# I2S9/dexterous-rl-manipulation

Hardware: NVIDIA B200
Metric: env_steps_per_sec (higher is better)
Workload: dtype f32+f64

## Files before the change

dexterous_rl_manipulation_b200/csrc/dexsim_kernels.cu:

```cuda
#include <cstdio>
#include <cstdlib>
#include <cstring>
#include <atomic>
#include <mutex>
#include <type_traits>

#include "dexsim_core.cuh"

namespace dexsim {

constexpr int STEP_MIN_BLOCKS = 2;
constexpr int STEP_THREADS = 256;

constexpr int SMEM_GROUPS_MAX = 64;

struct Hot {
    double op_old[3];
    float  ov_old[3];
    unsigned cmask_old;
};

__device__ __forceinline__ void load_env(const DexsimState& st, int64_t i, EnvRegs& e) {
    const int64_t ld = st.ld;
    const float* __restrict__ obs = st.obs;
// ... 80 lines not shown

__device__ __forceinline__ void record_episode(unsigned long long* cnt, double* rs, int success, int steps,
                                               int final_c, int la, int lb, int tie, double ret) {
    atomicAdd(&cnt[DEXSIM_CNT_EPISODES], 1ull);
    if (success) atomicAdd(&cnt[DEXSIM_CNT_SUCCESSES], 1ull);
    atomicAdd(&cnt[DEXSIM_CNT_SUM_STEPS], (unsigned long long)steps);
    atomicAdd(&cnt[DEXSIM_CNT_SUM_STEPS_SQ], (unsigned long long)steps * (unsigned long long)steps);
    if (final_c) atomicAdd(&cnt[DEXSIM_CNT_SUM_FINAL_CONTACTS], (unsigned long long)final_c);
    if (la != DEXSIM_LABEL_NONE) atomicAdd(&cnt[DEXSIM_CNT_LABEL_METRICS + la], 1ull);
    if (lb != DEXSIM_LABEL_NONE) atomicAdd(&cnt[DEXSIM_CNT_LABEL_TAXONOMY + lb], 1ull);
    if (tie == 1) atomicAdd(&cnt[DEXSIM_CNT_VAR_TIES], 1ull);
    if (rs) { atomicAdd(&rs[0], ret); atomicAdd(&rs[1], __dmul_rn(ret, ret)); }
}

struct EpisodeLog {
    DexsimEpisodeRecord* rec = nullptr;
    unsigned long long* count = nullptr;
    long long capacity = 0;
    uint32_t t_end = 0;
};

__device__ __forceinline__ void finish_episode(const EnvRegs& e, const DexsimParams& p, uint32_t gid, uint32_t episode,
                                               double ep_return, const EpStats& es, bool terminated, int n_c,
                                               unsigned long long* cnt, double* rs, const EpisodeLog* log,
                                               const bool classify = true) {
    if (!(cnt || (log && log->rec))) return;
    if (!classify) {
        if (cnt) record_episode(cnt, nullptr, p.success_is_terminated ? (terminated ? 1 : 0) : 0, e.sc, n_c,
                                DEXSIM_LABEL_NONE, DEXSIM_LABEL_NONE, 0, 0.0);
        return;
    }
    DexsimEpisodeSummary s;
    s.success = p.success_is_terminated ? (terminated ? 1 : 0) : 0;
    s.episode_steps = e.sc; s.num_contacts = n_c; s.final_contacts = n_c; s.hist_len = e.sc;
    int sum, sq, f5, l5, mx;
    epstats_unpack(es, sum, sq, f5, l5, mx);
    s.max_count = mx; s.sum_counts = sum; s.sum_sq_counts = sq; s.first5_sum = f5; s.last5_sum = l5;
    int la, lb, tie;
    classify_summary(s, p.loop_max_steps > 0 ? p.loop_max_steps : p.max_episode_steps, p.success_threshold, la, lb, tie);
    if (cnt) record_episode(cnt, rs, s.success, e.sc, n_c, la, lb, tie, ep_return);
    if (log && log->rec) {
        const unsigned long long slot = atomicAdd(log->count, 1ull);
        if ((long long)slot < log->capacity) {
            DexsimEpisodeRecord r;
            r.env_gid = gid; r.episode = episode; r.steps = e.sc;
            r.success = (uint8_t)s.success; r.final_contacts = (uint8_t)n_c;
            r.label_metrics = (uint8_t)la; r.label_taxonomy = (uint8_t)lb;
            r.episode_reward = ep_return; r.t_end = log->t_end; r.var_tie = (uint32_t)tie;
            log->rec[slot] = r;
        }
    }
}

__device__ __forceinline__ void finish_and_reset(EnvRegs& e, const DexsimParams& p, const DexsimGroup& grp,
                                                 uint32_t gid, uint32_t& episode, double& ep_return, EpStats& es,
                                                 bool terminated, int n_c, unsigned long long* cnt, double* rs,
                                                 double& size, double& mass, double& friction,
                                                 const EpisodeLog* log = nullptr, const bool classify = true) {
    finish_episode(e, p, gid, episode, ep_return, es, terminated, n_c, cnt, rs, log, classify);
    episode += 1u;
    float jp0[NJ], pos[3];
    reset_draws(p.seed, gid, episode, grp, jp0, size, mass, friction, pos);
    env_reset(e, jp0, size, friction, pos, !p.respawn);
    ep_return = 0.0;
    es.w0 = 0u; es.w1 = 0u;
}

__device__ __forceinline__ bool pending_reset(const EnvRegs& e, const DexsimParams& p) {
    return e.sc > 0 && (__popc(e.cmask) >= p.success_threshold || e.sc > p.max_episode_steps ||
                        (p.loop_max_steps > 0 && e.sc >= p.loop_max_steps));
}

__device__ __forceinline__ void next_step_reset(EnvRegs& e, const DexsimParams& p, const DexsimGroup& grp, uint32_t gid,
                                                uint32_t& episode, const DexsimState& st, int64_t i, StepResult& r) {
    double ep_return = 0.0, size, mass, friction;
    EpStats es{0u, 0u};
    finish_and_reset(e, p, grp, gid, episode, ep_return, es, false, 0, nullptr, nullptr, size, mass, friction);
    st.episode[i] = episode;
    st.size[i] = size; st.mass[i] = mass; st.friction[i] = friction;
    r.total = r.distance = r.contact = r.closure = r.stability = 0.0;
    r.n_c = __popc(e.cmask);
    r.terminated = r.truncated = false;
}

__device__ __forceinline__ float obs_entry(const EnvRegs& e, const int row) {
    if (row < DEXSIM_ROW_JV) return e.jp[row - DEXSIM_ROW_JP];
    if (row < DEXSIM_ROW_OP) return e.jv[row - DEXSIM_ROW_JV];
    if (row < DEXSIM_ROW_QUAT) return (float)e.op[row - DEXSIM_ROW_OP];
    if (row < DEXSIM_ROW_OV) return row == DEXSIM_ROW_QUAT ? 1.0f : 0.0f;
    if (row < DEXSIM_ROW_CONTACT) return e.ov[row - DEXSIM_ROW_OV];
    return ((e.cmask >> (row - DEXSIM_ROW_CONTACT)) & 1u) ? 1.0f : 0.0f;
}

}

#include "dexsim_step_tma.cuh"
#include "dexsim_rollout_split.cuh"

namespace dexsim {

template <bool TAGGED>
__device__ __forceinline__ void pack_env_body(const DexsimState& st, const DexsimStepIO& io, const int64_t i, const int after_reset,
                                              double* __restrict__ out) {
    const int t = threadIdx.x;
    const int64_t ld = st.ld;
    const bool noisy = io.noisy_obs && (io.obs_noise || io.sigma_obs != 0.0f);
    const float* obs = noisy ? io.noisy_obs : st.obs;
    if (t < NOBS) out[t] = (double)obs[t * ld + i];
    if (t == 45) out[45] = after_reset ? 0.0 : (io.reward64 ? io.reward64[i] : (double)io.reward[i]);
    if (t == 46) out[46] = after_reset ? 0.0 : (double)io.terminated[i];
    if (t == 47) out[47] = after_reset ? 0.0 : (double)io.truncated[i];
    if (t == 48) out[48] = (double)__popc((unsigned)st.cmask[i]);
    if (t == 49) out[49] = (double)st.step_count[i];
    if (t >= 50 && t < 53) out[t] = st.op64[(t - 50) * ld + i];
    if (t == 53) out[53] = st.size[i];
    if (t == 54) out[54] = st.mass[i];
    if (t == 55) out[55] = st.friction[i];
    if (t >= 56 && t < 60) out[t] = (io.reward_comps && !after_reset) ? (double)io.reward_comps[(t - 56) * ld + i] : 0.0;
// ... 700 lines not shown
    }
    if (need_groups) {
        if (p->num_groups < 1 || p->num_groups > DEXSIM_MAX_GROUPS) return DEXSIM_E_GROUPS;
        if (!groups) return DEXSIM_E_NULL;
    }
    return 0;
}

static int grid_for(int64_t n, int threads, int ctas_per_sm, int sm_count) {
    int64_t blocks = (n + threads - 1) / threads;
    const int64_t cap = (int64_t)sm_count * (ctas_per_sm > 0 ? ctas_per_sm : 1);
    if (blocks > cap) blocks = cap;
    if (blocks < 1) blocks = 1;
    return (int)blocks;
}

static inline int cuda_rc(cudaError_t e) { return e == cudaSuccess ? 0 : -(int)e; }

template <bool DENSE, bool AOS>
static void launch_step_variant(bool extras, bool next, int grid, cudaStream_t s, const DexsimState& st, const DexsimParams& p,
                                const DexsimGroup* groups, const uint16_t* goe, const DexsimStepIO& io,
                                double* pack_out, double pack_tag) {
    if (next)        step_kernel<DENSE, AOS, true, true><<<grid, STEP_THREADS, 0, s>>>(st, p, groups, goe, io, pack_out, pack_tag);
    else if (extras) step_kernel<DENSE, AOS, true, false><<<grid, STEP_THREADS, 0, s>>>(st, p, groups, goe, io, pack_out, pack_tag);
    else             step_kernel<DENSE, AOS, false, false><<<grid, STEP_THREADS, 0, s>>>(st, p, groups, goe, io);
}

template <auto KERNEL, typename GridOf, typename... Args>
static int launch_pdl(int threads, size_t smem, GridOf grid_of, cudaStream_t s, const Args&... args) {
    static thread_local int occupancy[64] = {0};
    int dev = 0;
    cudaError_t err = cudaGetDevice(&dev);
    if (err != cudaSuccess) return -(int)err;
    int uncached = 0;
    int& ctas_per_sm = (dev >= 0 && dev < 64) ? occupancy[dev] : uncached;
    if (ctas_per_sm == 0) {
        if (smem) {
            err = cudaFuncSetAttribute(KERNEL, cudaFuncAttributeMaxDynamicSharedMemorySize, (int)smem);
            if (err != cudaSuccess) return -(int)err;
        }
        err = cudaOccupancyMaxActiveBlocksPerMultiprocessor(&ctas_per_sm, KERNEL, threads, smem);
        if (err != cudaSuccess) return -(int)err;
        if (ctas_per_sm < 1) ctas_per_sm = 1;
    }
    cudaLaunchConfig_t cfg = {};
    cfg.gridDim = dim3((unsigned)grid_of(ctas_per_sm)); cfg.blockDim = dim3(threads); cfg.dynamicSmemBytes = smem; cfg.stream = s;
    cudaLaunchAttribute attr[1];
    attr[0].id = cudaLaunchAttributeProgrammaticStreamSerialization;
    attr[0].val.programmaticStreamSerializationAllowed = 1;
    cfg.attrs = attr; cfg.numAttrs = 1;
    return cuda_rc(cudaLaunchKernelEx(&cfg, KERNEL, args...));
}

template <bool DENSE, bool AOS, int TRACK, bool EXTRA, int STAGES, int TILE_, bool NEXT>
static int launch_tma_variant(int sm_count, cudaStream_t s, const DexsimState& st, const DexsimParams& p,
                              const DexsimGroup* groups, const uint16_t* goe, const DexsimStepIO& io,
                              const StepMaps& maps, int num_tiles) {
    constexpr int TMA_THREADS = TILE_ + 32;
    const size_t smem = (size_t)STAGES * StageLayout<TILE_>::stage_bytes(TRACK) + 2 * STAGES * (sizeof(uint64_t) + sizeof(int)) +
                        (TRACK ? TMA_GROUPS_MAX * (DEXSIM_NCOUNTERS * sizeof(unsigned long long) + 2 * sizeof(double)) : 0);
    return launch_pdl<step_tma_kernel<DENSE, AOS, TRACK, EXTRA, STAGES, TILE_, NEXT>>(
        TMA_THREADS, smem, [&](int ctas_per_sm) { return sm_count * ctas_per_sm < num_tiles ? sm_count * ctas_per_sm : num_tiles; }, s,
        st, p, groups, goe, io, maps, num_tiles, 1);
}

static int g_rollout_impl = 0;
static int g_step_impl = 0;

static int g_step_tile = 0;

static bool aligned16(const void* ptr) { return !(reinterpret_cast<uintptr_t>(ptr) & 15u); }

static int step_track(const DexsimState& st, const DexsimParams& p, const DexsimStepIO& io) {
    if (!p.auto_reset && st.ep_return == nullptr && io.finished == nullptr) return 0;
    return st.ep_return != nullptr ? 1 : 2;
}
static bool step_extra_io(const DexsimStepIO& io) {
    return io.dyn_noise || io.obs_noise || io.reward_comps || io.reward64 || io.sigma_dyn != 0.0f || io.sigma_obs != 0.0f;
}

static bool pipeline_eligible(const DexsimState& st, const DexsimStepIO& io, int track, bool extra_io, bool single) {
    return (!extra_io || io.action_layout == 1) && !single && st.n >= TILE && st.n < (int64_t)0x7FFFFF00 &&
           aligned16(io.action) && aligned16(io.reward) && aligned16(st.thr) && aligned16(st.damp) &&
           aligned16(st.step_count) && aligned16(st.cmask) && aligned16(io.terminated) && aligned16(io.truncated) &&
           aligned16(io.num_contacts) && aligned16(st.episode) && aligned16(io.finished) &&
           (track != 1 || (aligned16(st.ep_return) && aligned16(st.ep_stats))) &&
           g_step_impl != 1 && get_encode_fn() != nullptr;
}

static bool use_wide_tile(int64_t n, int track, int sm_count) {
    if (track == 1 || n < TILE_WIDE || TILE != 128) return false;
    if (g_step_tile) return g_step_tile == 2;
    if (n >= (int64_t)1 << 18) return false;
    auto depth = [](int64_t tiles, int64_t ctas) { return (int64_t)ceil((double)tiles / (double)ctas - 0.05); };
    const int64_t depth_narrow = depth((n + TILE - 1) / TILE, 3 * (int64_t)sm_count);
    const int64_t depth_wide = depth((n + TILE_WIDE - 1) / TILE_WIDE, 2 * (int64_t)sm_count);
    return depth_wide < depth_narrow;
}

static int launch_step_tma(const DexsimState* st, const DexsimParams* p, const DexsimGroup* groups, const uint16_t* goe,
                           const DexsimStepIO* io, cudaStream_t s, int track, bool extra, bool next, int sm_count) {
    struct MapCache { const void* obs; const void* op64; const void* act; const void* host; int64_t n, ld; int tile; bool valid; StepMaps maps; };
    static thread_local MapCache cache = {nullptr, nullptr, nullptr, nullptr, 0, 0, 0, false, {}};
    const bool aos = io->action_layout == 1;
    const bool wide = use_wide_tile(st->n, track, sm_count);
    const int tile = wide ? TILE_WIDE : TILE;
    const void* act_key = aos ? nullptr : (const void*)io->action;
    const void* host_key = (io->flags & DEXSIM_STEP_HOST_ALL_ROWS) ? (const void*)io->host_static_rows : nullptr;
    if (!(cache.valid && cache.obs == st->obs && cache.op64 == st->op64 && cache.act == act_key && cache.host == host_key &&
          cache.n == st->n && cache.ld == st->ld && cache.tile == tile)) {
        cache.valid = false;
        memset(&cache.maps, 0, sizeof(cache.maps));
        bool ok = make_map_2d(&cache.maps.obs_jpjv, CU_TENSOR_MAP_DATA_TYPE_FLOAT32, 4, st->obs, st->n, st->ld, DEXSIM_OBS, 30, tile) &&
                  make_map_2d(&cache.maps.obs_ov, CU_TENSOR_MAP_DATA_TYPE_FLOAT32, 4, st->obs, st->n, st->ld, DEXSIM_OBS, 3, tile) &&
                  make_map_2d(&cache.maps.op64, CU_TENSOR_MAP_DATA_TYPE_FLOAT64, 8, st->op64, st->n, st->ld, 3, 3, tile);
        if (ok && !aos)
            ok = make_map_2d(&cache.maps.act_soa, CU_TENSOR_MAP_DATA_TYPE_FLOAT32, 4, const_cast<float*>(io->action), st->n,
                             st->ld, NJ, NJ, tile);
        if (ok && host_key)
            ok = make_map_2d(&cache.maps.host_jpjv, CU_TENSOR_MAP_DATA_TYPE_FLOAT32, 4, const_cast<void*>(host_key), st->n, st->ld,
                             DEXSIM_OBS, 30, tile);
        if (!ok) return 1;
        cache.obs = st->obs; cache.op64 = st->op64; cache.act = act_key; cache.host = host_key; cache.n = st->n; cache.ld = st->ld; cache.tile = tile;
        cache.valid = true;
    }
    const StepMaps& maps = cache.maps;
    const int num_tiles = (int)((st->n + tile - 1) / tile);
    const auto as_bool = [](bool b, auto&& f) { return b ? f(std::true_type{}) : f(std::false_type{}); };
    const auto as_track = [](int t, auto&& f) {
        using std::integral_constant;
        return t == 1 ? f(integral_constant<int, 1>{}) : t == 2 ? f(integral_constant<int, 2>{}) : f(integral_constant<int, 0>{});
    };
    return as_bool(p->reward_type == 1, [&](auto dense) {
        return as_bool(aos, [&](auto aos_) {
            return as_track(track, [&](auto track_) {
                return as_bool(extra, [&](auto extra_) {
                    return as_bool(next, [&](auto next_) -> int {
                        constexpr bool DENSE = decltype(dense)::value, AOS = decltype(aos_)::value, EXTRA = decltype(extra_)::value;
                        constexpr int TRACK = decltype(track_)::value;
                        constexpr bool NEXT = decltype(next_)::value;
                        if constexpr ((EXTRA && !AOS) || (NEXT && TRACK == 0)) {
                            return 1;
                        } else {
                            if constexpr (TRACK != 1) {
                                if (wide)
                                    return launch_tma_variant<DENSE, AOS, TRACK, EXTRA, 2, TILE_WIDE, NEXT>(sm_count, s, *st, *p,
                                                                                                            groups, goe, *io, maps,
                                                                                                            num_tiles);
                            }
                            return launch_tma_variant<DENSE, AOS, TRACK, EXTRA, DEXSIM_TMA_STAGES, TILE, NEXT>(sm_count, s, *st, *p,
                                                                                                               groups, goe, *io,
                                                                                                               maps, num_tiles);
                        }
                    });
                });
            });
        });
    });
}

static int launch_step(const DexsimState* st, const DexsimParams* p, const DexsimGroup* groups,
                       const uint16_t* goe, const DexsimStepIO* io, cudaStream_t s,
                       double* pack_out = nullptr, double pack_tag = 0.0, bool next = false) {
    int rc = check_state(st);
    if (rc) return rc;
    if (!io || !io->action || !io->reward || !io->terminated || !io->truncated || !io->num_contacts) return DEXSIM_E_NULL;
    if (io->action_layout != 0 && io->action_layout != 1) return DEXSIM_E_PARAM;
    const bool fused_dyn = !io->dyn_noise && io->sigma_dyn != 0.0f;
    const bool fused_obs = !io->obs_noise && io->sigma_obs != 0.0f;
    if ((io->obs_noise != nullptr || fused_obs) != (io->noisy_obs != nullptr)) return DEXSIM_E_NULL;
    if (pack_out && st->n != 1) return DEXSIM_E_SIZE;
    const bool extras = io->dyn_noise || io->obs_noise || io->reward_comps || io->reward64 || io->finished || io->host_static_rows ||
                        (p && p->auto_reset) || st->ep_return != nullptr || fused_dyn || fused_obs || pack_out != nullptr;
    const bool group_sigma = (fused_dyn && io->sigma_dyn < 0.0f) || (fused_obs && io->sigma_obs < 0.0f);
    rc = check_params(p, p && (p->auto_reset || group_sigma), groups, st->ep_return != nullptr && p && p->auto_reset);
    if (rc) return rc;
    if (st->n == 0) return 0;
    DeviceInfo di;
    rc = device_info_cached(di);
    if (rc) return rc;
    const int track = step_track(*st, *p, *io);
    const bool extra_io = step_extra_io(*io);
    if (pipeline_eligible(*st, *io, track, extra_io, pack_out != nullptr)) {
        rc = launch_step_tma(st, p, groups, goe, io, s, track, extra_io, next, di.sm_count);
        if (rc <= 0) return rc;
    }
    if (g_step_impl == 2) return DEXSIM_E_PARAM;
    if (io->flags & DEXSIM_STEP_HOST_ALL_ROWS) return DEXSIM_E_PARAM;
    const int grid = grid_for(st->n, STEP_THREADS, di.step_ctas, di.sm_count);
    const bool dense = p->reward_type == 1, aos = io->action_layout == 1;
    if (dense) { if (aos) launch_step_variant<true, true>(extras, next, grid, s, *st, *p, groups, goe, *io, pack_out, pack_tag);
                 else     launch_step_variant<true, false>(extras, next, grid, s, *st, *p, groups, goe, *io, pack_out, pack_tag); }
    else       { if (aos) launch_step_variant<false, true>(extras, next, grid, s, *st, *p, groups, goe, *io, pack_out, pack_tag);
                 else     launch_step_variant<false, false>(extras, next, grid, s, *st, *p, groups, goe, *io, pack_out, pack_tag); }
    return cuda_rc(cudaGetLastError());
}
// ... 631 lines not shown
```

dexterous_rl_manipulation_b200/csrc/dexsim_step_tma.cuh:

```cuda
#pragma once

#include <cuda.h>

#include "dexsim_core.cuh"

namespace dexsim {

#ifndef DEXSIM_TMA_TILE
#define DEXSIM_TMA_TILE 128
#endif
#ifndef DEXSIM_TMA_STAGES
#define DEXSIM_TMA_STAGES 2
#endif
constexpr int TILE = DEXSIM_TMA_TILE;
constexpr int TILE_WIDE = 224;
static_assert(TILE % 32 == 0 && TILE <= 256, "a tile is a whole number of warps and one TMA box wide");
constexpr int TMA_GROUPS_MAX = 16;

template <int T>
struct StageLayout {
    static_assert(T % 32 == 0 && T <= 256, "a tile is a whole number of warps and one TMA box wide");
    static constexpr int OFF_JPJV = 0;
    static constexpr int OFF_OV = OFF_JPJV + 30 * T * 4;
    static constexpr int OFF_OP64 = OFF_OV + 3 * T * 4;
    static constexpr int OFF_THR = OFF_OP64 + 3 * T * 8;
    static constexpr int OFF_ACT = OFF_THR + T * 8;
    static constexpr int OFF_DAMP = OFF_ACT + NJ * T * 4;
    static constexpr int OFF_SC = OFF_DAMP + T * 4;
    static constexpr int OFF_REWARD = OFF_SC + T * 4;
    static constexpr int OFF_CMASK = OFF_REWARD + T * 4;
    static constexpr int OFF_TERM = OFF_CMASK + T;
    static constexpr int OFF_TRUNC = OFF_TERM + T;
    static constexpr int OFF_NC = OFF_TRUNC + T;
    static constexpr int OFF_FIN = OFF_NC + T;
    static constexpr int OFF_EPISODE = OFF_FIN + T;
    static constexpr int OFF_EPRET = OFF_EPISODE + T * 4;
    static constexpr int OFF_EPST0 = OFF_EPRET + T * 8;
    static constexpr int OFF_EPST1 = OFF_EPST0 + T * 4;
    __host__ __device__ static constexpr int stage_bytes(int track) {
        return ((track == 1 ? OFF_EPST1 + T * 4 : OFF_EPRET) + 127) / 128 * 128;
    }
    static_assert(OFF_OV % 128 == 0 && OFF_OP64 % 128 == 0 && OFF_ACT % 128 == 0, "tensor-map box destinations");
    static_assert(OFF_THR % 16 == 0 && OFF_DAMP % 16 == 0 && OFF_SC % 16 == 0 && OFF_REWARD % 16 == 0 && OFF_CMASK % 16 == 0 &&
                  OFF_TERM % 16 == 0 && OFF_TRUNC % 16 == 0 && OFF_NC % 16 == 0 && OFF_EPRET % 16 == 0 && OFF_EPST0 % 16 == 0 &&
                  OFF_EPST1 % 16 == 0 && OFF_FIN % 16 == 0 && OFF_EPISODE % 16 == 0, "1-D bulk copy destinations");
};

struct StepMaps {
    CUtensorMap obs_jpjv;
    CUtensorMap obs_ov;
    CUtensorMap op64;
    CUtensorMap act_soa;
    CUtensorMap host_jpjv;
};

__device__ __forceinline__ uint32_t smem_u32(const void* p) { return (uint32_t)__cvta_generic_to_shared(p); }

__device__ __forceinline__ void mbar_init(uint32_t bar, uint32_t count) {
    asm volatile("mbarrier.init.shared::cta.b64 [%0], %1;" ::"r"(bar), "r"(count));
}
__device__ __forceinline__ void mbar_expect_tx(uint32_t bar, uint32_t bytes) {
    asm volatile("mbarrier.arrive.expect_tx.shared::cta.b64 _, [%0], %1;" ::"r"(bar), "r"(bytes) : "memory");
}
__device__ __forceinline__ void mbar_arrive(uint32_t bar) {
    asm volatile("mbarrier.arrive.shared::cta.b64 _, [%0];" ::"r"(bar) : "memory");
}
__device__ __forceinline__ void mbar_wait(uint32_t bar, uint32_t parity) {
    uint32_t ok = 0;
    while (!ok) {
        asm volatile("{ .reg .pred p; mbarrier.try_wait.parity.shared::cta.b64 p, [%1], %2; selp.u32 %0, 1, 0, p; }"
                     : "=r"(ok) : "r"(bar), "r"(parity) : "memory");
    }
}
__device__ __forceinline__ void tma_load_2d(uint32_t dst, const CUtensorMap* map, int c0, int c1, uint32_t bar) {
    asm volatile("cp.async.bulk.tensor.2d.shared::cluster.global.mbarrier::complete_tx::bytes [%0], [%1, {%2, %3}], [%4];"
                 ::"r"(dst), "l"(map), "r"(c0), "r"(c1), "r"(bar) : "memory");
}
__device__ __forceinline__ void tma_store_2d(const CUtensorMap* map, int c0, int c1, uint32_t src) {
    asm volatile("cp.async.bulk.tensor.2d.global.shared::cta.bulk_group [%0, {%1, %2}], [%3];"
                 ::"l"(map), "r"(c0), "r"(c1), "r"(src) : "memory");
}
__device__ __forceinline__ void bulk_load(uint32_t dst, const void* src, uint32_t bytes, uint32_t bar) {
    asm volatile("cp.async.bulk.shared::cluster.global.mbarrier::complete_tx::bytes [%0], [%1], %2, [%3];"
                 ::"r"(dst), "l"(src), "r"(bytes), "r"(bar) : "memory");
}
__device__ __forceinline__ void bulk_store(void* dst, uint32_t src, uint32_t bytes) {
    asm volatile("cp.async.bulk.global.shared::cta.bulk_group [%0], [%1], %2;" ::"l"(dst), "r"(src), "r"(bytes) : "memory");
}
__device__ __forceinline__ void bulk_commit() { asm volatile("cp.async.bulk.commit_group;" ::: "memory"); }
__device__ __forceinline__ void bulk_wait_read0() { asm volatile("cp.async.bulk.wait_group.read 0;" ::: "memory"); }
__device__ __forceinline__ void bulk_wait0() { asm volatile("cp.async.bulk.wait_group 0;" ::: "memory"); }
__device__ __forceinline__ void fence_async_smem() { asm volatile("fence.proxy.async.shared::cta;" ::: "memory"); }

template <int T>
__device__ __forceinline__ uint32_t tile_cols(int64_t n, int64_t base) {
    const int64_t left = n - base;
    return left >= T ? (uint32_t)T : (uint32_t)((left + 31) & ~(int64_t)31);
}


template <bool DENSE, bool AOS, int TRACK, bool EXTRA, int STAGES, int TILE_, bool NEXT>
__global__ void __launch_bounds__(TILE_ + 32, (STAGES == 2) ? (TILE_ <= 96 ? 4 : (TILE_ >= 192 ? 2 : 3)) : (STAGES == 1 ? 4 : 2))
step_tma_kernel(const DexsimState st, const DexsimParams p, const DexsimGroup* __restrict__ groups,
                const uint16_t* __restrict__ group_of_env, const DexsimStepIO io,
                const __grid_constant__ StepMaps maps, const int num_tiles, const int pdl) {
    constexpr int TILE = TILE_;
    static_assert(TRACK != 1 || TILE_ <= 128, "the full-tracking arrays only fit the narrow tile's stages");
    static_assert(!NEXT || TRACK != 0, "next-step auto-reset needs the episode bookkeeping of TRACK 1 or 2");
    using SL = StageLayout<TILE_>;
    constexpr int OFF_JPJV = SL::OFF_JPJV, OFF_OV = SL::OFF_OV, OFF_OP64 = SL::OFF_OP64, OFF_THR = SL::OFF_THR, OFF_ACT = SL::OFF_ACT,
                  OFF_DAMP = SL::OFF_DAMP, OFF_SC = SL::OFF_SC, OFF_REWARD = SL::OFF_REWARD, OFF_CMASK = SL::OFF_CMASK,
                  OFF_TERM = SL::OFF_TERM, OFF_TRUNC = SL::OFF_TRUNC, OFF_NC = SL::OFF_NC, OFF_FIN = SL::OFF_FIN,
                  OFF_EPISODE = SL::OFF_EPISODE, OFF_EPRET = SL::OFF_EPRET, OFF_EPST0 = SL::OFF_EPST0, OFF_EPST1 = SL::OFF_EPST1;
    (void)OFF_EPRET; (void)OFF_EPST0; (void)OFF_EPST1; (void)OFF_ACT;
    constexpr int STAGE_BYTES = SL::stage_bytes(TRACK);
    constexpr int TMA_COMPUTE_THREADS = TILE;
    constexpr int TMA_THREADS = TMA_COMPUTE_THREADS + 32;
    extern __shared__ __align__(1024) unsigned char smem[];
    unsigned char* stage_base = smem;
    uint64_t* bars = reinterpret_cast<uint64_t*>(smem + STAGES * STAGE_BYTES);
    int* s_tile = reinterpret_cast<int*>(bars + 2 * STAGES);
    unsigned long long* sh_cnt = reinterpret_cast<unsigned long long*>(s_tile + 2 * STAGES);
    double* sh_rs = reinterpret_cast<double*>(sh_cnt + (TRACK ? TMA_GROUPS_MAX * DEXSIM_NCOUNTERS : 0));

    constexpr int PRODUCER_TID = TMA_COMPUTE_THREADS;
    const int tid = threadIdx.x;
    const int64_t n = st.n, ld = st.ld;
    const bool count_episodes = TRACK && p.auto_reset && io.counters != nullptr;
    const bool staged_cnt = count_episodes && p.num_groups <= TMA_GROUPS_MAX;
    const bool host_all = (io.flags & DEXSIM_STEP_HOST_ALL_ROWS) != 0 && io.host_static_rows != nullptr;
    const bool load_episode = (EXTRA && ((!io.dyn_noise && io.sigma_dyn != 0.0f) || (!io.obs_noise && io.noisy_obs && io.sigma_obs != 0.0f))) ||
                              (TRACK && p.auto_reset);

    if (tid == 0) {
        for (int b = 0; b < STAGES; ++b) mbar_init(smem_u32(&bars[b]), 1);
        for (int b = 0; b < STAGES; ++b) mbar_init(smem_u32(&bars[STAGES + b]), TMA_COMPUTE_THREADS);
        asm volatile("fence.mbarrier_init.release.cluster;" ::: "memory");
    }
    if (TRACK && staged_cnt) {
        for (int w = tid; w < p.num_groups * DEXSIM_NCOUNTERS; w += TMA_THREADS) sh_cnt[w] = 0ull;
        for (int w = tid; w < p.num_groups * 2; w += TMA_THREADS) sh_rs[w] = 0.0;
    }
    __syncthreads();

    if (pdl) asm volatile("griddepcontrol.launch_dependents;" ::: "memory");
    if (tid >= PRODUCER_TID) {
        if (tid == PRODUCER_TID) {
            if (pdl) asm volatile("griddepcontrol.wait;" ::: "memory");
            unsigned int* sched = io.sched;
            auto issue_stores = [&](int s, int tile) {
                const int64_t base = (int64_t)tile * TILE;
                const uint32_t sb = smem_u32(stage_base + (size_t)s * STAGE_BYTES);
                const uint32_t cols = tile_cols<TILE>(n, base);
                tma_store_2d(&maps.obs_jpjv, (int)base, DEXSIM_ROW_JP, sb + OFF_JPJV);
                if (host_all) {
                    tma_store_2d(&maps.host_jpjv, (int)base, DEXSIM_ROW_JP, sb + OFF_JPJV);
                    bulk_store(io.host_static_rows + (int64_t)(DEXSIM_ROW_OP + 2) * ld + base, sb + OFF_OV, cols * 4);
                    bulk_store(io.host_static_rows + (int64_t)(DEXSIM_ROW_OV + 2) * ld + base, sb + OFF_OV + 2 * TILE * 4, cols * 4);
                    if (io.host_cmask) bulk_store(io.host_cmask + base, sb + OFF_CMASK, cols);
                }
                bulk_store(st.step_count + base, sb + OFF_SC, cols * 4);
                bulk_store(io.reward + base, sb + OFF_REWARD, cols * 4);
                bulk_store(io.terminated + base, sb + OFF_TERM, cols);
                bulk_store(io.truncated + base, sb + OFF_TRUNC, cols);
                bulk_store(io.num_contacts + base, sb + OFF_NC, cols);
                if (TRACK == 1) {
                    bulk_store(st.ep_return + base, sb + OFF_EPRET, cols * 8);
                    bulk_store(st.ep_stats + base, sb + OFF_EPST0, cols * 4);
                    bulk_store(st.ep_stats + ld + base, sb + OFF_EPST1, cols * 4);
                }
                if (TRACK && io.finished) bulk_store(io.finished + base, sb + OFF_FIN, cols);
                bulk_commit();
            };
            unsigned held = 0u;
            const bool reverse = (io.flags & DEXSIM_STEP_REVERSE_TILES) != 0;
            int tile = (int)blockIdx.x;
            int k = 0;
            for (;; ++k) {
                const int s = k % STAGES, use = k / STAGES;
                const uint32_t sb = smem_u32(stage_base + (size_t)s * STAGE_BYTES);
                const uint32_t full = smem_u32(&bars[s]);
                if ((held >> s) & 1u) {
                    mbar_wait(smem_u32(&bars[STAGES + s]), (uint32_t)((use - 1) & 1));
                    issue_stores(s, s_tile[s]);
                    held &= ~(1u << s);
                    bulk_wait_read0();
                }
                if (tile >= num_tiles) {
                    s_tile[s] = -1;
                    mbar_arrive(full);
                    break;
                }
                const int tile_id = reverse ? num_tiles - 1 - tile : tile;
                s_tile[s] = tile_id;
                held |= 1u << s;
                const int64_t base = (int64_t)tile_id * TILE;
                const uint32_t cols = tile_cols<TILE>(n, base);
                const bool full_tile = (n - base) >= TILE;
                uint32_t tx = (30 + 3) * TILE * 4 + 3 * TILE * 8 + cols * (8 + 4 + 4 + 1);
                if (AOS) tx += full_tile ? NJ * TILE * 4 : 0;
                else tx += NJ * TILE * 4;
                if (TRACK == 1) tx += cols * (8 + 4 + 4);
                if (load_episode) tx += cols * 4;
                mbar_expect_tx(full, tx);
                tma_load_2d(sb + OFF_JPJV, &maps.obs_jpjv, (int)base, DEXSIM_ROW_JP, full);
                tma_load_2d(sb + OFF_OV, &maps.obs_ov, (int)base, DEXSIM_ROW_OV, full);
                tma_load_2d(sb + OFF_OP64, &maps.op64, (int)base, 0, full);
                if (AOS) { if (full_tile) bulk_load(sb + OFF_ACT, io.action + base * NJ, NJ * TILE * 4, full); }
                else tma_load_2d(sb + OFF_ACT, &maps.act_soa, (int)base, 0, full);
                bulk_load(sb + OFF_THR, st.thr + base, cols * 8, full);
                bulk_load(sb + OFF_DAMP, st.damp + base, cols * 4, full);
                bulk_load(sb + OFF_SC, st.step_count + base, cols * 4, full);
                bulk_load(sb + OFF_CMASK, st.cmask + base, cols, full);
                if (TRACK == 1) {
                    bulk_load(sb + OFF_EPRET, st.ep_return + base, cols * 8, full);
                    bulk_load(sb + OFF_EPST0, st.ep_stats + base, cols * 4, full);
                    bulk_load(sb + OFF_EPST1, st.ep_stats + ld + base, cols * 4, full);
                }
                if (load_episode) bulk_load(sb + OFF_EPISODE, st.episode + base, cols * 4, full);
                tile = sched ? (int)(atomicAdd(&sched[0], 1u) + gridDim.x) : tile + (int)gridDim.x;
            }
            for (int d = 1; d < STAGES; ++d) {
                const int kk = k - STAGES + d;
                if (kk < 0) continue;
                const int s = kk % STAGES;
                if (!((held >> s) & 1u)) continue;
                mbar_wait(smem_u32(&bars[STAGES + s]), (uint32_t)((kk / STAGES) & 1));
                issue_stores(s, s_tile[s]);
            }
            bulk_wait0();
            if (sched) {
                __threadfence();
                if (atomicAdd(&sched[1], 1u) == gridDim.x - 1) { sched[0] = 0u; sched[1] = 0u; }
            }
        }
    } else {
        const int col = tid;
        for (int k = 0;; ++k) {
            const int s = k % STAGES;
            unsigned char* sp = stage_base + (size_t)s * STAGE_BYTES;
            mbar_wait(smem_u32(&bars[s]), (uint32_t)((k / STAGES) & 1));
            const int tile = s_tile[s];
            if (tile < 0) break;
            const int64_t base = (int64_t)tile * TILE;
            const int64_t i = base + col;
            float* s_jpjv = reinterpret_cast<float*>(sp + OFF_JPJV);
            double* s_op = reinterpret_cast<double*>(sp + OFF_OP64);
            float* __restrict__ obs = st.obs;
            const bool valid = i < n;
            bool lane_reset = false;
            bool fused_dyn = false, fused_obs = false;
            uint32_t episode = 0u;
            int g = 0;
            EnvRegs e;
            if (valid) {
                const float* s_ov = reinterpret_cast<const float*>(sp + OFF_OV);
#pragma unroll
                for (int j = 0; j < NJ; ++j) { e.jp[j] = s_jpjv[j * TILE + col]; e.jv[j] = s_jpjv[(NJ + j) * TILE + col]; }
#pragma unroll
                for (int c = 0; c < 3; ++c) { e.ov[c] = s_ov[c * TILE + col]; e.op[c] = s_op[c * TILE + col]; }
                e.thr = reinterpret_cast<const double*>(sp + OFF_THR)[col];
                e.damp = reinterpret_cast<const float*>(sp + OFF_DAMP)[col];
                e.sc = reinterpret_cast<const int*>(sp + OFF_SC)[col];
                e.cmask = reinterpret_cast<const uint8_t*>(sp + OFF_CMASK)[col];
                bool pending = false;
                if constexpr (NEXT) pending = pending_reset(e, p);
                float a[NJ];
                const float* s_act = reinterpret_cast<const float*>(sp + OFF_ACT);
                if (AOS) {
                    if ((n - base) >= TILE) {
#pragma unroll
                        for (int j = 0; j < NJ; ++j) a[j] = s_act[col * NJ + j];
                    } else {
#pragma unroll
                        for (int j = 0; j < NJ; ++j) a[j] = __ldg(io.action + i * NJ + j);
                    }
                } else {
#pragma unroll
                    for (int j = 0; j < NJ; ++j) a[j] = s_act[j * TILE + col];
                }
                const int64_t gid = p.env_gid0 + i;
                if (EXTRA) {
                    fused_dyn = !io.dyn_noise && io.sigma_dyn != 0.0f;
                    fused_obs = !io.obs_noise && io.noisy_obs && io.sigma_obs != 0.0f;
                    if (fused_dyn || fused_obs) {
                        episode = reinterpret_cast<const uint32_t*>(sp + OFF_EPISODE)[col];
                        if (io.sigma_dyn < 0.0f || io.sigma_obs < 0.0f)
                            g = group_of_env ? (int)group_of_env[i] : (int)((uint32_t)gid % (uint32_t)p.num_groups);
                    }
                    if (io.dyn_noise) {
#pragma unroll
                        for (int j = 0; j < NJ; ++j)
                            a[j] = clip_f32(__fadd_rn(a[j], __ldg(io.dyn_noise + j * ld + i)), -1.0f, 1.0f);
                    } else if (fused_dyn && !pending) {
                        const float sigma = io.sigma_dyn > 0.0f ? io.sigma_dyn : groups[g].sigma_dyn;
                        if (sigma > 0.0f) {
                            float nz[NJ];
                            normal_rows<NJ>(p.seed, (uint32_t)gid, episode, (uint32_t)e.sc, STREAM_DYN, sigma, nz);
#pragma unroll
                            for (int j = 0; j < NJ; ++j) a[j] = clip_f32(__fadd_rn(a[j], nz[j]), -1.0f, 1.0f);
                        }
                    }
                }
                double op_old[3]; float ov_old[3];
#pragma unroll
                for (int c = 0; c < 3; ++c) { op_old[c] = e.op[c]; ov_old[c] = e.ov[c]; }
                const unsigned cmask_old = e.cmask;

                StepResult r;
                if constexpr (NEXT) {
                    if (pending) {
                        g = group_of_env ? (int)group_of_env[i] : (int)((uint32_t)gid % (uint32_t)p.num_groups);
                        episode = reinterpret_cast<const uint32_t*>(sp + OFF_EPISODE)[col];
                        next_step_reset(e, p, groups[g], (uint32_t)gid, episode, st, i, r);
                        st.thr[i] = e.thr; st.damp[i] = e.damp;
                    } else {
                        env_step<DENSE>(e, a, p, r);
                    }
                } else {
                    env_step<DENSE>(e, a, p, r);
                }

                reinterpret_cast<float*>(sp + OFF_REWARD)[col] = (float)r.total;
                (sp + OFF_TERM)[col] = r.terminated ? 1 : 0;
                (sp + OFF_TRUNC)[col] = r.truncated ? 1 : 0;
                (sp + OFF_NC)[col] = (unsigned char)r.n_c;
                if (EXTRA) {
                    if (io.reward64) io.reward64[i] = r.total;
                    if (io.reward_comps) {
                        io.reward_comps[0 * ld + i] = (float)r.distance;
                        io.reward_comps[1 * ld + i] = (float)r.contact;
                        io.reward_comps[2 * ld + i] = (float)r.closure;
                        io.reward_comps[3 * ld + i] = (float)r.stability;
                    }
                }

                if (TRACK) {
                    double ep_return = 0.0;
                    EpStats es{0u, 0u};
                    if (TRACK == 1 && !pending) {
                        ep_return = __dadd_rn(reinterpret_cast<double*>(sp + OFF_EPRET)[col], r.total);
                        es.w0 = reinterpret_cast<uint32_t*>(sp + OFF_EPST0)[col];
                        es.w1 = reinterpret_cast<uint32_t*>(sp + OFF_EPST1)[col];
                        epstats_push(es, e.sc - 1, r.n_c);
                    }
                    const bool done = r.terminated || r.truncated || (p.loop_max_steps > 0 && e.sc >= p.loop_max_steps);
                    if (p.auto_reset && done) {
                        g = group_of_env ? (int)group_of_env[i] : (int)((uint32_t)gid % (uint32_t)p.num_groups);
                        episode = reinterpret_cast<const uint32_t*>(sp + OFF_EPISODE)[col];
                        unsigned long long* cnt = nullptr;
                        double* rs = nullptr;
                        if (count_episodes) {
                            cnt = (staged_cnt ? sh_cnt : reinterpret_cast<unsigned long long*>(io.counters)) + (int64_t)g * DEXSIM_NCOUNTERS;
                            if (io.ret_sums) rs = (staged_cnt ? sh_rs : io.ret_sums) + 2 * g;
                        }
                        if constexpr (NEXT) {
                            finish_episode(e, p, (uint32_t)gid, episode, ep_return, es, r.terminated, r.n_c, cnt, rs, nullptr,
                                           TRACK == 1);
                            lane_reset = true;
                        } else
                        {
                            double size, mass, friction;
                            finish_and_reset(e, p, groups[g], (uint32_t)gid, episode, ep_return, es, r.terminated, r.n_c,
                                             cnt, rs, size, mass, friction, nullptr, TRACK == 1);
                            st.episode[i] = episode;
                            st.size[i] = size; st.mass[i] = mass; st.friction[i] = friction;
                            st.thr[i] = e.thr; st.damp[i] = e.damp;
                            lane_reset = true;
                        }
                    }
                    if (TRACK == 1) {
                        reinterpret_cast<double*>(sp + OFF_EPRET)[col] = ep_return;
                        reinterpret_cast<uint32_t*>(sp + OFF_EPST0)[col] = es.w0;
                        reinterpret_cast<uint32_t*>(sp + OFF_EPST1)[col] = es.w1;
                    }
                    (sp + OFF_FIN)[col] = lane_reset ? 1 : 0;
                }
                {
#pragma unroll
                    for (int j = 0; j < NJ; ++j) { s_jpjv[j * TILE + col] = e.jp[j]; s_jpjv[(NJ + j) * TILE + col] = e.jv[j]; }
                    reinterpret_cast<int*>(sp + OFF_SC)[col] = e.sc;
#pragma unroll
                    for (int c = 0; c < 3; ++c) {
                        if (__double_as_longlong(e.op[c]) != __double_as_longlong(op_old[c])) {
                            st.op64[c * ld + i] = e.op[c];
                            obs[(DEXSIM_ROW_OP + c) * ld + i] = (float)e.op[c];
                            if (c < 2 && io.host_static_rows) io.host_static_rows[(DEXSIM_ROW_OP + c) * ld + i] = (float)e.op[c];
                        }
                        if (__float_as_uint(e.ov[c]) != __float_as_uint(ov_old[c])) {
                            obs[(DEXSIM_ROW_OV + c) * ld + i] = e.ov[c];
                            if (c < 2 && io.host_static_rows) io.host_static_rows[(DEXSIM_ROW_OV + c) * ld + i] = e.ov[c];
                        }
                    }
                    if (host_all) {
                        float* s_out = reinterpret_cast<float*>(sp + OFF_OV);
                        s_out[col] = (float)e.op[2];
                        s_out[2 * TILE + col] = e.ov[2];
                        (sp + OFF_CMASK)[col] = (uint8_t)e.cmask;
                    }
                    const unsigned flip = e.cmask ^ cmask_old;
                    if (flip) {
#pragma unroll
                        for (int f = 0; f < NF; ++f)
                            if ((flip >> f) & 1u) obs[(DEXSIM_ROW_CONTACT + f) * ld + i] = ((e.cmask >> f) & 1u) ? 1.0f : 0.0f;
                        st.cmask[i] = (uint8_t)e.cmask;
                    }
                }
            }
            if (EXTRA && valid && io.noisy_obs) {
                float* __restrict__ out = io.noisy_obs;
                if (io.obs_noise) {
                    const float* __restrict__ nz = io.obs_noise;
#pragma unroll
                    for (int row = 0; row < NOBS; ++row)
                        out[row * ld + i] = __fadd_rn(obs_entry(e, row), __ldg(nz + row * ld + i));
                } else if (fused_obs) {
                    const float sigma = io.sigma_obs > 0.0f ? io.sigma_obs : groups[g].sigma_obs;
                    const int64_t gid = p.env_gid0 + i;
#pragma unroll
                    for (int b = 0; b < (NOBS + 3) / 4; ++b) {
                        const U4 o = rng_block(p.seed, (uint32_t)gid, episode, (uint32_t)e.sc, STREAM_OBS, (uint32_t)b);
                        float z[4];
                        normal_pair(o.x, o.y, z[0], z[1]);
                        normal_pair(o.z, o.w, z[2], z[3]);
#pragma unroll
                        for (int q = 0; q < 4; ++q) {
                            const int row = 4 * b + q;
                            if (row < NOBS) out[row * ld + i] = __fadd_rn(obs_entry(e, row), __fmul_rn(sigma, z[q]));
                        }
                    }
                }
            }
            fence_async_smem();
            mbar_arrive(smem_u32(&bars[STAGES + s]));
        }
    }
    if (TRACK && staged_cnt) {
        __syncthreads();
        unsigned long long* gc = reinterpret_cast<unsigned long long*>(io.counters);
        for (int w = tid; w < p.num_groups * DEXSIM_NCOUNTERS; w += TMA_THREADS)
            if (sh_cnt[w]) atomicAdd(&gc[w], sh_cnt[w]);
        if (io.ret_sums)
            for (int w = tid; w < p.num_groups * 2; w += TMA_THREADS)
                if (sh_rs[w] != 0.0) atomicAdd(&io.ret_sums[w], sh_rs[w]);
    }
}

typedef CUresult (*EncodeTiledFn)(CUtensorMap*, CUtensorMapDataType, cuuint32_t, void*, const cuuint64_t*,
                                  const cuuint64_t*, const cuuint32_t*, const cuuint32_t*, CUtensorMapInterleave,
                                  CUtensorMapSwizzle, CUtensorMapL2promotion, CUtensorMapFloatOOBfill);

static EncodeTiledFn get_encode_fn() {
    static EncodeTiledFn fn = nullptr;
    static bool tried = false;
    if (!tried) {
        tried = true;
        void* sym = nullptr;
        cudaDriverEntryPointQueryResult q;
        if (cudaGetDriverEntryPoint("cuTensorMapEncodeTiled", &sym, cudaEnableDefault, &q) == cudaSuccess &&
            q == cudaDriverEntryPointSuccess)
            fn = reinterpret_cast<EncodeTiledFn>(sym);
    }
    return fn;
}

static bool make_map_2d(CUtensorMap* m, CUtensorMapDataType dt, size_t elem, void* base, int64_t n, int64_t ld,
                        int rows, int box_rows, int tile) {
    EncodeTiledFn enc = get_encode_fn();
    if (!enc) return false;
    const cuuint64_t dims[2] = {(cuuint64_t)n, (cuuint64_t)rows};
    const cuuint64_t strides[1] = {(cuuint64_t)ld * elem};
    const cuuint32_t box[2] = {(cuuint32_t)tile, (cuuint32_t)box_rows};
    const cuuint32_t estr[2] = {1, 1};
    return enc(m, dt, 2, base, dims, strides, box, estr, CU_TENSOR_MAP_INTERLEAVE_NONE, CU_TENSOR_MAP_SWIZZLE_NONE,
               CU_TENSOR_MAP_L2_PROMOTION_L2_256B, CU_TENSOR_MAP_FLOAT_OOB_FILL_NONE) == CUDA_SUCCESS;
}

}
```

Measured before the change: 18.43 billion.

## Defer auto-reset of finished envs to a batched post-pass via shared-memory list

Auto-reset work for finished environments is taken out of the per-lane step path. Each finished env index is appended to a shared-memory list using a warp ballot and an atomic. The reset draws and state writes run later in batches: when the list nears capacity the producer drains the in-flight tiles and inserts a sentinel stage, and a final pass handles whatever remains after the loop. This targets warp divergence from the costly reset path and drops the per-tile episode load. In exchange it adds larger dynamic shared memory, extra synchronization and pipeline drains, and relies on global-proxy fence ordering between TMA stores and the generic-proxy reset stores.

```diff
diff --git a/dexterous_rl_manipulation_b200/csrc/dexsim_kernels.cu b/dexterous_rl_manipulation_b200/csrc/dexsim_kernels.cu
--- a/dexterous_rl_manipulation_b200/csrc/dexsim_kernels.cu
+++ b/dexterous_rl_manipulation_b200/csrc/dexsim_kernels.cu
@@ -156,18 +156,51 @@
     }
 }
 
+__device__ __forceinline__ void next_episode(EnvRegs& e, const DexsimParams& p, const DexsimGroup& grp, uint32_t gid,
+                                             uint32_t& episode, double& size, double& mass, double& friction) {
+    episode += 1u;
+    float jp0[NJ], pos[3];
+    reset_draws(p.seed, gid, episode, grp, jp0, size, mass, friction, pos);
+    env_reset(e, jp0, size, friction, pos, !p.respawn);
+}
+
 __device__ __forceinline__ void finish_and_reset(EnvRegs& e, const DexsimParams& p, const DexsimGroup& grp,
                                                  uint32_t gid, uint32_t& episode, double& ep_return, EpStats& es,
                                                  bool terminated, int n_c, unsigned long long* cnt, double* rs,
                                                  double& size, double& mass, double& friction,
                                                  const EpisodeLog* log = nullptr, const bool classify = true) {
     finish_episode(e, p, gid, episode, ep_return, es, terminated, n_c, cnt, rs, log, classify);
-    episode += 1u;
-    float jp0[NJ], pos[3];
-    reset_draws(p.seed, gid, episode, grp, jp0, size, mass, friction, pos);
-    env_reset(e, jp0, size, friction, pos, !p.respawn);
+    next_episode(e, p, grp, gid, episode, size, mass, friction);
     ep_return = 0.0;
     es.w0 = 0u; es.w1 = 0u;
+}
+
+struct FinishedReset {
+    EnvRegs e;
+    double size, mass, friction;
+    uint32_t episode;
+};
+__device__ __forceinline__ void draw_finished_reset(const DexsimState& st, const DexsimParams& p, const DexsimGroup* __restrict__ groups,
+                                                    const uint16_t* __restrict__ group_of_env, int64_t i, FinishedReset& r) {
+    const int64_t gid = p.env_gid0 + i;
+    const int g = group_index(group_of_env, i, gid, p.num_groups);
+    if (!p.respawn) {
+#pragma unroll
+        for (int k = 0; k < 3; ++k) r.e.op[k] = st.op64[k * st.ld + i];
+    }
+    r.episode = st.episode[i];
+    next_episode(r.e, p, groups[g], (uint32_t)gid, r.episode, r.size, r.mass, r.friction);
+}
+__device__ __forceinline__ void store_finished_reset(const DexsimState& st, int64_t i, const FinishedReset& r, float* host) {
+    st.episode[i] = r.episode;
+    st.size[i] = r.size; st.mass[i] = r.mass; st.friction[i] = r.friction;
+    store_env_full(st, i, r.e, host);
+}
+__device__ __forceinline__ void reset_finished_env(const DexsimState& st, const DexsimParams& p, const DexsimGroup* __restrict__ groups,
+                                                   const uint16_t* __restrict__ group_of_env, int64_t i, float* host) {
+    FinishedReset r;
+    draw_finished_reset(st, p, groups, group_of_env, i, r);
+    store_finished_reset(st, i, r, host);
 }
 
 __device__ __forceinline__ bool pending_reset(const EnvRegs& e, const DexsimParams& p) {
@@ -974,14 +1007,13 @@
     return cuda_rc(cudaLaunchKernelEx(&cfg, KERNEL, args...));
 }
 
-template <bool DENSE, bool AOS, int TRACK, bool EXTRA, int STAGES, int TILE_, bool NEXT>
+template <bool DENSE, bool AOS, int TRACK, bool EXTRA, int STAGES, int TILE_, bool NEXT, bool DEFER = false>
 static int launch_tma_variant(int sm_count, cudaStream_t s, const DexsimState& st, const DexsimParams& p,
                               const DexsimGroup* groups, const uint16_t* goe, const DexsimStepIO& io,
                               const StepMaps& maps, int num_tiles) {
     constexpr int TMA_THREADS = TILE_ + 32;
-    const size_t smem = (size_t)STAGES * StageLayout<TILE_>::stage_bytes(TRACK) + 2 * STAGES * (sizeof(uint64_t) + sizeof(int)) +
-                        (TRACK ? TMA_GROUPS_MAX * (DEXSIM_NCOUNTERS * sizeof(unsigned long long) + 2 * sizeof(double)) : 0);
-    return launch_pdl<step_tma_kernel<DENSE, AOS, TRACK, EXTRA, STAGES, TILE_, NEXT>>(
+    const size_t smem = (size_t)TmaSmem<TILE_, STAGES, TRACK>::bytes(DEFER);
+    return launch_pdl<step_tma_kernel<DENSE, AOS, TRACK, EXTRA, STAGES, TILE_, NEXT, DEFER>>(
         TMA_THREADS, smem, [&](int ctas_per_sm) { return sm_count * ctas_per_sm < num_tiles ? sm_count * ctas_per_sm : num_tiles; }, s,
         st, p, groups, goe, io, maps, num_tiles, 1);
 }
@@ -1048,6 +1080,7 @@
     }
     const StepMaps& maps = cache.maps;
     const int num_tiles = (int)((st->n + tile - 1) / tile);
+    const bool defer = track != 0 && p->auto_reset && !extra && !next && !(io->flags & DEXSIM_STEP_HOST_ALL_ROWS);
     const auto as_bool = [](bool b, auto&& f) { return b ? f(std::true_type{}) : f(std::false_type{}); };
     const auto as_track = [](int t, auto&& f) {
         using std::integral_constant;
@@ -1064,6 +1097,17 @@
                         if constexpr ((EXTRA && !AOS) || (NEXT && TRACK == 0)) {
                             return 1;
                         } else {
+                            if constexpr (TRACK != 0 && !EXTRA && !NEXT) {
+                                if (defer) {
+                                    if constexpr (TRACK != 1) {
+                                        if (wide)
+                                            return launch_tma_variant<DENSE, AOS, TRACK, false, 2, TILE_WIDE, false, true>(
+                                                sm_count, s, *st, *p, groups, goe, *io, maps, num_tiles);
+                                    }
+                                    return launch_tma_variant<DENSE, AOS, TRACK, false, DEXSIM_TMA_STAGES, TILE, false, true>(
+                                        sm_count, s, *st, *p, groups, goe, *io, maps, num_tiles);
+                                }
+                            }
                             if constexpr (TRACK != 1) {
                                 if (wide)
                                     return launch_tma_variant<DENSE, AOS, TRACK, EXTRA, 2, TILE_WIDE, NEXT>(sm_count, s, *st, *p,
diff --git a/dexterous_rl_manipulation_b200/csrc/dexsim_step_tma.cuh b/dexterous_rl_manipulation_b200/csrc/dexsim_step_tma.cuh
--- a/dexterous_rl_manipulation_b200/csrc/dexsim_step_tma.cuh
+++ b/dexterous_rl_manipulation_b200/csrc/dexsim_step_tma.cuh
@@ -46,6 +46,16 @@
                   OFF_EPST1 % 16 == 0 && OFF_FIN % 16 == 0 && OFF_EPISODE % 16 == 0, "1-D bulk copy destinations");
 };
 
+template <int T, int STAGES, int TRACK>
+struct TmaSmem {
+    static constexpr int CTAS_PER_SM = (STAGES == 2) ? (T <= 96 ? 4 : (T >= 192 ? 2 : 3)) : (STAGES == 1 ? 4 : 2);
+    static constexpr int BASE = STAGES * StageLayout<T>::stage_bytes(TRACK) + 2 * STAGES * (8 + 4) +
+                                (TRACK ? TMA_GROUPS_MAX * (DEXSIM_NCOUNTERS * 8 + 2 * 8) : 0);
+    static constexpr int LIST_HEADER = 16;
+    static constexpr int LIST_CAP = (228 * 1024 / CTAS_PER_SM - 1024 - (BASE + LIST_HEADER + 127) / 128 * 128) / 1024 * 256;
+    static constexpr int bytes(bool defer) { return BASE + (defer ? LIST_HEADER + 4 * LIST_CAP : 0); }
+};
+
 struct StepMaps {
     CUtensorMap obs_jpjv;
     CUtensorMap obs_ov;
@@ -91,6 +101,7 @@
 __device__ __forceinline__ void bulk_wait_read0() { asm volatile("cp.async.bulk.wait_group.read 0;" ::: "memory"); }
 __device__ __forceinline__ void bulk_wait0() { asm volatile("cp.async.bulk.wait_group 0;" ::: "memory"); }
 __device__ __forceinline__ void fence_async_smem() { asm volatile("fence.proxy.async.shared::cta;" ::: "memory"); }
+__device__ __forceinline__ void fence_async_global() { asm volatile("fence.proxy.async.global;" ::: "memory"); }
 
 template <int T>
 __device__ __forceinline__ uint32_t tile_cols(int64_t n, int64_t base) {
@@ -99,14 +110,17 @@
 }
 
 
-template <bool DENSE, bool AOS, int TRACK, bool EXTRA, int STAGES, int TILE_, bool NEXT>
-__global__ void __launch_bounds__(TILE_ + 32, (STAGES == 2) ? (TILE_ <= 96 ? 4 : (TILE_ >= 192 ? 2 : 3)) : (STAGES == 1 ? 4 : 2))
+template <bool DENSE, bool AOS, int TRACK, bool EXTRA, int STAGES, int TILE_, bool NEXT, bool DEFER = false>
+__global__ void __launch_bounds__(TILE_ + 32, (TmaSmem<TILE_, STAGES, TRACK>::CTAS_PER_SM))
 step_tma_kernel(const DexsimState st, const DexsimParams p, const DexsimGroup* __restrict__ groups,
                 const uint16_t* __restrict__ group_of_env, const DexsimStepIO io,
                 const __grid_constant__ StepMaps maps, const int num_tiles, const int pdl) {
     constexpr int TILE = TILE_;
     static_assert(TRACK != 1 || TILE_ <= 128, "the full-tracking arrays only fit the narrow tile's stages");
     static_assert(!NEXT || TRACK != 0, "next-step auto-reset needs the episode bookkeeping of TRACK 1 or 2");
+    static_assert(!DEFER || (TRACK != 0 && !EXTRA && !NEXT), "the deferred auto-reset is the plain auto-reset step's");
+    constexpr int LIST_CAP = TmaSmem<TILE_, STAGES, TRACK>::LIST_CAP;
+    static_assert(!DEFER || LIST_CAP >= STAGES * TILE_, "the reset list takes the tiles in flight after it is emptied");
     using SL = StageLayout<TILE_>;
     constexpr int OFF_JPJV = SL::OFF_JPJV, OFF_OV = SL::OFF_OV, OFF_OP64 = SL::OFF_OP64, OFF_THR = SL::OFF_THR, OFF_ACT = SL::OFF_ACT,
                   OFF_DAMP = SL::OFF_DAMP, OFF_SC = SL::OFF_SC, OFF_REWARD = SL::OFF_REWARD, OFF_CMASK = SL::OFF_CMASK,
@@ -122,15 +136,17 @@
     int* s_tile = reinterpret_cast<int*>(bars + 2 * STAGES);
     unsigned long long* sh_cnt = reinterpret_cast<unsigned long long*>(s_tile + 2 * STAGES);
     double* sh_rs = reinterpret_cast<double*>(sh_cnt + (TRACK ? TMA_GROUPS_MAX * DEXSIM_NCOUNTERS : 0));
+    int* s_nlist = reinterpret_cast<int*>(sh_rs + (TRACK ? TMA_GROUPS_MAX * 2 : 0));
+    int* s_list = s_nlist + TmaSmem<TILE_, STAGES, TRACK>::LIST_HEADER / 4;
 
     constexpr int PRODUCER_TID = TMA_COMPUTE_THREADS;
     const int tid = threadIdx.x;
     const int64_t n = st.n, ld = st.ld;
     const bool count_episodes = TRACK && p.auto_reset && io.counters != nullptr;
     const bool staged_cnt = count_episodes && p.num_groups <= TMA_GROUPS_MAX;
-    const bool host_all = (io.flags & DEXSIM_STEP_HOST_ALL_ROWS) != 0 && io.host_static_rows != nullptr;
+    const bool host_all = !DEFER && (io.flags & DEXSIM_STEP_HOST_ALL_ROWS) != 0 && io.host_static_rows != nullptr;
     const bool load_episode = (EXTRA && ((!io.dyn_noise && io.sigma_dyn != 0.0f) || (!io.obs_noise && io.noisy_obs && io.sigma_obs != 0.0f))) ||
-                              (TRACK && p.auto_reset);
+                              (TRACK && p.auto_reset && !DEFER);
 
     if (tid == 0) {
         for (int b = 0; b < STAGES; ++b) mbar_init(smem_u32(&bars[b]), 1);
@@ -141,9 +157,12 @@
         for (int w = tid; w < p.num_groups * DEXSIM_NCOUNTERS; w += TMA_THREADS) sh_cnt[w] = 0ull;
         for (int w = tid; w < p.num_groups * 2; w += TMA_THREADS) sh_rs[w] = 0.0;
     }
+    if (DEFER && tid == 0) *s_nlist = 0;
     __syncthreads();
 
     if (pdl) asm volatile("griddepcontrol.launch_dependents;" ::: "memory");
+    int listed = 0;
+    FinishedReset first;
     if (tid >= PRODUCER_TID) {
         if (tid == PRODUCER_TID) {
             if (pdl) asm volatile("griddepcontrol.wait;" ::: "memory");
@@ -185,6 +204,24 @@
                     issue_stores(s, s_tile[s]);
                     held &= ~(1u << s);
                     bulk_wait_read0();
+                }
+                if (DEFER && tile < num_tiles && *reinterpret_cast<volatile int*>(s_nlist) + STAGES * TILE > LIST_CAP) {
+                    for (int d = 1; d < STAGES; ++d) {
+                        const int kk = k - STAGES + d;
+                        if (kk < 0) continue;
+                        const int s2 = kk % STAGES;
+                        if (!((held >> s2) & 1u)) continue;
+                        mbar_wait(smem_u32(&bars[STAGES + s2]), (uint32_t)((kk / STAGES) & 1));
+                        issue_stores(s2, s_tile[s2]);
+                        held &= ~(1u << s2);
+                    }
+                    bulk_wait0();
+                    fence_async_global();
+                    s_tile[s] = -2;
+                    mbar_arrive(full);
+                    mbar_wait(smem_u32(&bars[STAGES + s]), (uint32_t)(use & 1));
+                    *s_nlist = 0;
+                    continue;
                 }
                 if (tile >= num_tiles) {
                     s_tile[s] = -1;
@@ -229,6 +266,7 @@
                 issue_stores(s, s_tile[s]);
             }
             bulk_wait0();
+            if (DEFER) fence_async_global();
             if (sched) {
                 __threadfence();
                 if (atomicAdd(&sched[1], 1u) == gridDim.x - 1) { sched[0] = 0u; sched[1] = 0u; }
@@ -241,6 +279,13 @@
             unsigned char* sp = stage_base + (size_t)s * STAGE_BYTES;
             mbar_wait(smem_u32(&bars[s]), (uint32_t)((k / STAGES) & 1));
             const int tile = s_tile[s];
+            if (DEFER && tile == -2) {
+                const int n_listed = *s_nlist;
+                for (int j = col; j < n_listed; j += TILE)
+                    reset_finished_env(st, p, groups, group_of_env, (int64_t)s_list[j], io.host_static_rows);
+                mbar_arrive(smem_u32(&bars[STAGES + s]));
+                continue;
+            }
             if (tile < 0) break;
             const int64_t base = (int64_t)tile * TILE;
             const int64_t i = base + col;
@@ -347,7 +392,7 @@
                     const bool done = r.terminated || r.truncated || (p.loop_max_steps > 0 && e.sc >= p.loop_max_steps);
                     if (p.auto_reset && done) {
                         g = group_of_env ? (int)group_of_env[i] : (int)((uint32_t)gid % (uint32_t)p.num_groups);
-                        episode = reinterpret_cast<const uint32_t*>(sp + OFF_EPISODE)[col];
+                        if (!DEFER) episode = reinterpret_cast<const uint32_t*>(sp + OFF_EPISODE)[col];
                         unsigned long long* cnt = nullptr;
                         double* rs = nullptr;
                         if (count_episodes) {
@@ -357,6 +402,12 @@
                         if constexpr (NEXT) {
                             finish_episode(e, p, (uint32_t)gid, episode, ep_return, es, r.terminated, r.n_c, cnt, rs, nullptr,
                                            TRACK == 1);
+                            lane_reset = true;
+                        } else if constexpr (DEFER) {
+                            finish_episode(e, p, (uint32_t)gid, 0u, ep_return, es, r.terminated, r.n_c, cnt, rs, nullptr,
+                                           TRACK == 1);
+                            ep_return = 0.0;
+                            es.w0 = 0u; es.w1 = 0u;
                             lane_reset = true;
                         } else
                         {
@@ -431,8 +482,30 @@
                     }
                 }
             }
+            if constexpr (DEFER) {
+                const unsigned m = __ballot_sync(0xffffffffu, lane_reset);
+                if (m) {
+                    const int lane = col & 31, leader = __ffs(m) - 1;
+                    int at = 0;
+                    if (lane == leader) at = atomicAdd(s_nlist, __popc(m));
+                    at = __shfl_sync(0xffffffffu, at, leader);
+                    if (lane_reset) s_list[at + __popc(m & ((1u << lane) - 1u))] = (int)i;
+                }
+            }
             fence_async_smem();
             mbar_arrive(smem_u32(&bars[STAGES + s]));
+        }
+        if constexpr (DEFER) {
+            asm volatile("bar.sync 1, %0;" ::"r"(TMA_COMPUTE_THREADS) : "memory");
+            listed = *s_nlist;
+            if (col < listed) draw_finished_reset(st, p, groups, group_of_env, (int64_t)s_list[col], first);
+        }
+    }
+    if constexpr (DEFER) {
+        __syncthreads();
+        for (int j = tid; j < listed; j += TMA_COMPUTE_THREADS) {
+            if (j == tid) store_finished_reset(st, (int64_t)s_list[j], first, io.host_static_rows);
+            else reset_finished_env(st, p, groups, group_of_env, (int64_t)s_list[j], io.host_static_rows);
         }
     }
     if (TRACK && staged_cnt) {
```

Measured after the change: 18.25 billion (median of 6 runs). No clear change (-1.0%).
